# iostanin1/SCTL

Hardware: AMD Instinct MI355X
Metric: pair-interactions/s, Laplace-SL N x N direct sum (higher is better)
Workload: dtype f64; 1 GPU; Laplace3D single layer (Laplace3D-FxU), 2^20 x 2^20, fp64 [BASELINE headline / north_star target]; kernel=Laplace3D-FxU, n_trg=1048576, n_src=1048576, digits=-1

## Files before the change

sctl_amd/csrc/centered.hip:

```cpp
#include "centered_kernel.hpp"
#include "centered_mfma_kernel.hpp"
#include <sctl_amd/device/launch.hpp>
#include "workspace.hpp"

#include <cstdlib>

#include <rocprim/device/device_radix_sort.hpp>

namespace sctl_amd {

#define CENTERED_TRY(expr)            \
  do {                                \
    hipError_t e_ = (expr);           \
    if (e_ != hipSuccess) return e_;  \
  } while (0)


namespace {
bool use_mfma_f32() {
  const char* e = std::getenv("SCTL_AMD_MFMA_F32");
  return !(e && e[0] == '0');
}
}
int centered_pipe(int kernel_id, int real, int mode) {
  const bool has = kernel_id == Laplace3D_FxU::ID || kernel_id == Laplace3D_DxU::ID || kernel_id == Stokes3D_FxU::ID || kernel_id == Stokes3D_FSxU::ID ||
                   kernel_id == Stokes3D_FxUP::ID || kernel_id == Stokes3D_DxU::ID || kernel_id == Stokes3D_FxT::ID || kernel_id == Laplace3D_FxdU::ID || kernel_id == Laplace3D_FDxUdU::ID;
  return (has && real == 1  && mode == 0 && use_mfma_f32()) ? 2 : 1;
}
int centered_targets_per_wave(int kernel_id, int real, int mode, int64_t density) {
  if (centered_pipe(kernel_id, real, mode) != 2) {
    if (kernel_id == Laplace3D_FxdU::ID) return 64 * CenteredFxdU<double>::targets_per_lane<double>();
    if (kernel_id == Stokes3D_FxUP::ID) return 64 * CenteredStokeslet<double, Stokes3D_FxUP>::targets_per_lane<double>();
    return 64 * (real == 0  ? CenteredFxU<double>::targets_per_lane<double>() : CenteredFxU<float>::targets_per_lane<float>());
  }
  if (const char* e = (kernel_id == Laplace3D_FxU::ID || kernel_id == Laplace3D_DxU::ID) ? std::getenv("SCTL_AMD_MFMA_CB") : nullptr) {
    if (e[0] == '8') return 256;
    if (e[0] == '4') return 128;
  }
  if (kernel_id != Laplace3D_FxU::ID && kernel_id != Laplace3D_DxU::ID) return 128;
  return (kernel_id == Laplace3D_FxU::ID && density < ((int64_t)1 << 20)) ? 128 : 256;
}
namespace {
template <class R> struct CenteredStresslet { using Ker = Stokes3D_DxU; };
template <class CP> struct mfma_moments_policy { using type = void; };
template <class KER> struct mfma_moments_policy<CenteredStokeslet<float, KER>> { using type = MfmaStokeslet<KER>; };
template <> struct mfma_moments_policy<CenteredStresslet<float>> { using type = MfmaStresslet; };
template <class R> struct CenteredTraction { using Ker = Stokes3D_FxT; };
template <class R> struct CenteredFusedLaplace { using Ker = Laplace3D_FDxUdU; };
template <> struct mfma_moments_policy<CenteredFusedLaplace<float>> { using type = MfmaFusedLaplace; };
template <> struct mfma_moments_policy<CenteredFxdU<float>> { using type = MfmaGradient; };
template <> struct mfma_moments_policy<CenteredTraction<float>> { using type = MfmaTraction; };
template <class CP, class R, int MODE> void launch_centered(const EvalArgs<R>& a, dim3 grid, int per_wave, hipStream_t st) {
  using MP = typename mfma_moments_policy<CP>::type;
  if constexpr (std::is_same<R, float>::value && !std::is_void<MP>::value) {
    if constexpr (MODE == 0) hipLaunchKernelGGL((centered_mfma_moments_f32_kernel<MP>), grid, dim3(kWaveBlock), 0, st, a);
    return;
  } else {
  if constexpr (std::is_same<R, float>::value && MODE == 0) {
    if (use_mfma_f32()) {
      constexpr bool DL = std::is_same<CP, CenteredDxU<float>>::value;
      if (per_wave == 256) {
        if constexpr (DL) hipLaunchKernelGGL((centered_mfma_f32_kernel<true, 8>), grid, dim3(kWaveBlock), 0, st, a);
        else hipLaunchKernelGGL(centered_mfma_fxu256_f32_kernel, grid, dim3(kWaveBlock), 0, st, a);
      } else {
        hipLaunchKernelGGL((centered_mfma_f32_kernel<DL, 4>), grid, dim3(kWaveBlock), 0, st, a);
      }
      return;
    }
  }
  hipLaunchKernelGGL((centered_kernel<CP, R, MODE, CP::template targets_per_lane<R>()>), grid, dim3(kWaveBlock), 0, st, a);
  }
}
}

void centered_plan(int64_t Nt, int64_t Ns, int cus, int src_bytes, int out_bytes, int* T, int* splits, int64_t* chunk) {
  *T = 2;
  const int64_t wg_x = (Nt + kWaveBlock * 2 - 1) / (kWaveBlock * 2);
  const int64_t want = (int64_t)cus * 16 * 64;
  const int64_t ntile = (Ns + kWaveTile - 1) / kWaveTile;
  int64_t s = (want + wg_x - 1) / wg_x;
  const int64_t s_l2 = (Ns * src_bytes + (2 << 20) - 1) / (2 << 20);
  if (s < s_l2) s = s_l2;
  if (s > ntile / 64) s = ntile / 64;
  if (s > 8) s = (s + 7) & ~(int64_t)7;
  if (s > 256) s = 256;
  {
    const int64_t fit = ((int64_t)2 << 30) / (Nt * out_bytes > 0 ? Nt * out_bytes : 1);
    if (s > fit) s = (fit >= 8) ? (fit & ~(int64_t)7) : fit;
  }
  if (s < 1) s = 1;
  const int64_t tiles_per = (ntile + s - 1) / s;
  *chunk = tiles_per * kWaveTile;
  *splits = (int)((Ns + *chunk - 1) / *chunk);
}

template <class CP, class R>
hipError_t eval_centered_t(int64_t Nt, int64_t Ns, const R* xt, const R* xs, const R* xn, const R* f, R* v_trg, double scale_d, int mode, int cus,
                           hipStream_t st, bool presorted, int64_t density) {
  const R scale = (R)scale_d;
  constexpr int K1 = CP::Ker::K1;
  int T, splits;
  int64_t chunk;
  centered_plan(Nt, Ns, cus, (int)sizeof(R) * (3 + CP::Ker::ND + CP::Ker::K0), (int)sizeof(R) * K1, &T, &splits, &chunk);
  if (presorted) {
    R* partial = nullptr;
    if (splits > 1) {
      void* base = nullptr;
      CENTERED_TRY(workspace_acquire(st, sizeof(R) * (size_t)splits * (size_t)Nt * K1, &base));
      partial = (R*)base;
    }
    EvalArgs<R> a{};
    a.Nt = Nt; a.Ns = Ns; a.xt = xt; a.xs = xs; a.xn = xn; a.f = f; a.v_trg = v_trg; a.partial = partial;
    a.chunk = chunk; a.scale = scale;
    a.ctx.v[0] = kNearFactor2;
    const int64_t per_wave = centered_targets_per_wave(CP::Ker::ID, sizeof(R) == 8 ? 0 : 1, mode, density);
    const dim3 grid((unsigned)((Nt + per_wave - 1) / per_wave), (unsigned)splits);
    if (mode == 0) launch_centered<CP, R, 0>(a, grid, (int)per_wave, st);
    else if (mode == 1) launch_centered<CP, R, 1>(a, grid, (int)per_wave, st);
    else launch_centered<CP, R, (sizeof(R) == 8 ? 2 : 1)>(a, grid, (int)per_wave, st);
    CENTERED_TRY(hipGetLastError());
    if (splits > 1)
      hipLaunchKernelGGL((reduce_splits_kernel<R>), dim3((unsigned)((Nt * K1 + kBlock - 1) / kBlock)), dim3(kBlock), 0, st, v_trg, (const R*)partial, Nt * K1, splits, scale);
    return hipGetLastError();
  }
  const int nblk_box = 256;
  const unsigned nb = (unsigned)((Nt + kBlock - 1) / kBlock);
  size_t tmp_bytes = 0;
  CENTERED_TRY(rocprim::radix_sort_pairs(nullptr, tmp_bytes, (uint64_t*)nullptr, (uint64_t*)nullptr, (uint32_t*)nullptr, (uint32_t*)nullptr, (size_t)Nt, 0,
                                         63, st));
  const size_t n = (size_t)Nt;
  const size_t total = Carver::pad(sizeof(double) * 6 * nblk_box) + 2 * Carver::pad(sizeof(uint64_t) * n) + 2 * Carver::pad(sizeof(uint32_t) * n) +
                       Carver::pad(sizeof(R) * 3 * n) + Carver::pad(sizeof(R) * n * K1) + Carver::pad(tmp_bytes) +
                       (splits > 1 ? Carver::pad(sizeof(R) * (size_t)splits * n * K1) : 0);
  void* base = nullptr;
  CENTERED_TRY(workspace_acquire(st, total, &base));
  Carver cut(base);
  double* part = cut.take<double>(6 * nblk_box);
  uint64_t *keys = cut.take<uint64_t>(n), *keys2 = cut.take<uint64_t>(n);
  uint32_t *idx = cut.take<uint32_t>(n), *idx2 = cut.take<uint32_t>(n);
  R *xts = cut.take<R>(3 * n), *outs = cut.take<R>(n * K1);
  char* tmp = cut.take<char>(tmp_bytes);
  R* partial = (splits > 1) ? cut.take<R>((size_t)splits * n * K1) : nullptr;

  hipLaunchKernelGGL((bbox_partial_kernel<R>), dim3(nblk_box), dim3(kBlock), 0, st, xt, Nt, part);
  hipLaunchKernelGGL((morton_keys_kernel<R>), dim3(nb), dim3(kBlock), 0, st, xt, Nt, (const double*)part, nblk_box, keys, idx);
  CENTERED_TRY(rocprim::radix_sort_pairs(tmp, tmp_bytes, keys, keys2, idx, idx2, (size_t)Nt, 0, 63, st));
  const uint32_t* perm = idx2;
  hipLaunchKernelGGL((gather_points_kernel<R>), dim3(nb), dim3(kBlock), 0, st, xt, perm, Nt, xts);
  CENTERED_TRY(hipMemsetAsync(outs, 0, sizeof(R) * Nt * K1, st));

  EvalArgs<R> a{};
  a.Nt = Nt; a.Ns = Ns; a.xt = xts; a.xs = xs; a.xn = xn; a.f = f; a.v_trg = outs; a.partial = nullptr;
  a.chunk = chunk; a.scale = scale;
  a.ctx.v[0] = kNearFactor2;
  a.partial = partial;
  const int64_t per_wave = centered_targets_per_wave(CP::Ker::ID, sizeof(R) == 8 ? 0 : 1, mode, density);
  const dim3 grid((unsigned)((Nt + per_wave - 1) / per_wave), (unsigned)splits);
  if (mode == 0) launch_centered<CP, R, 0>(a, grid, (int)per_wave, st);
  else if (mode == 1) launch_centered<CP, R, 1>(a, grid, (int)per_wave, st);
  else launch_centered<CP, R, (sizeof(R) == 8 ? 2 : 1)>(a, grid, (int)per_wave, st);
  CENTERED_TRY(hipGetLastError());
  if (splits > 1)
    hipLaunchKernelGGL((reduce_splits_kernel<R>), dim3((unsigned)((Nt * K1 + kBlock - 1) / kBlock)), dim3(kBlock), 0, st, outs, (const R*)a.partial, Nt * K1, splits, scale);
  hipLaunchKernelGGL((scatter_add_kernel<R>), dim3(nb), dim3(kBlock), 0, st, (const R*)outs, perm, Nt, K1, v_trg);
  return hipGetLastError();
}
template <class R> hipError_t morton_order_device_t(const R* d_x, int64_t n, R* d_sorted, uint32_t* d_perm, hipStream_t st) {
  if (n <= 0) return hipSuccess;
  const int nblk_box = 256;
  const unsigned nb = (unsigned)((n + kBlock - 1) / kBlock);
  size_t tmp_bytes = 0;
  CENTERED_TRY(rocprim::radix_sort_pairs(nullptr, tmp_bytes, (uint64_t*)nullptr, (uint64_t*)nullptr, (uint32_t*)nullptr, (uint32_t*)nullptr, (size_t)n, 0, 63, st));
  const size_t total = Carver::pad(sizeof(double) * 6 * nblk_box) + 2 * Carver::pad(sizeof(uint64_t) * (size_t)n) + Carver::pad(sizeof(uint32_t) * (size_t)n) + Carver::pad(tmp_bytes);
  void* base = nullptr;
  CENTERED_TRY(workspace_acquire(st, total, &base));
  Carver cut(base);
  double* part = cut.take<double>(6 * nblk_box);
  uint64_t *keys = cut.take<uint64_t>((size_t)n), *keys2 = cut.take<uint64_t>((size_t)n);
  uint32_t* idx = cut.take<uint32_t>((size_t)n);
  char* tmp = cut.take<char>(tmp_bytes);
  hipLaunchKernelGGL((bbox_partial_kernel<R>), dim3(nblk_box), dim3(kBlock), 0, st, d_x, n, part);
  hipLaunchKernelGGL((morton_keys_kernel<R>), dim3(nb), dim3(kBlock), 0, st, d_x, n, (const double*)part, nblk_box, keys, idx);
  CENTERED_TRY(rocprim::radix_sort_pairs(tmp, tmp_bytes, keys, keys2, idx, d_perm, (size_t)n, 0, 63, st));
  hipLaunchKernelGGL((gather_points_kernel<R>), dim3(nb), dim3(kBlock), 0, st, d_x, (const uint32_t*)d_perm, n, d_sorted);
  return hipGetLastError();
}
hipError_t morton_order_device(int real, const void* d_x, int64_t n, void* d_sorted, uint32_t* d_perm, hipStream_t st) {
  return real == 0  ? morton_order_device_t<double>((const double*)d_x, n, (double*)d_sorted, d_perm, st)
                              : morton_order_device_t<float>((const float*)d_x, n, (float*)d_sorted, d_perm, st);
}

template <class R>
hipError_t eval_centered(int kernel_id, int64_t Nt, int64_t Ns, const R* xt, const R* xs, const R* xn, const R* f, R* v_trg, double scale, int mode, int cus,
                         hipStream_t st, bool presorted, int64_t density) {
  if (kernel_id == Laplace3D_DxU::ID) return eval_centered_t<CenteredDxU<R>, R>(Nt, Ns, xt, xs, xn, f, v_trg, scale, mode, cus, st, presorted, density);
  if constexpr (std::is_same<R, double>::value) {
    if (kernel_id == Laplace3D_FxdU::ID) return eval_centered_t<CenteredFxdU<R>, R>(Nt, Ns, xt, xs, xn, f, v_trg, scale, mode, cus, st, presorted, density);
    if (kernel_id == Stokes3D_FxUP::ID) return eval_centered_t<CenteredStokeslet<R, Stokes3D_FxUP>, R>(Nt, Ns, xt, xs, xn, f, v_trg, scale, mode, cus, st, presorted, density);
  }
  if constexpr (std::is_same<R, float>::value) {
    if (kernel_id == Laplace3D_FxdU::ID) return eval_centered_t<CenteredFxdU<R>, R>(Nt, Ns, xt, xs, xn, f, v_trg, scale, mode, cus, st, presorted, density);
    if (kernel_id == Laplace3D_FDxUdU::ID) return eval_centered_t<CenteredFusedLaplace<R>, R>(Nt, Ns, xt, xs, xn, f, v_trg, scale, mode, cus, st, presorted, density);
    if (kernel_id == Stokes3D_FxU::ID) return eval_centered_t<CenteredStokeslet<R, Stokes3D_FxU>, R>(Nt, Ns, xt, xs, xn, f, v_trg, scale, mode, cus, st, presorted, density);
    if (kernel_id == Stokes3D_FSxU::ID) return eval_centered_t<CenteredStokeslet<R, Stokes3D_FSxU>, R>(Nt, Ns, xt, xs, xn, f, v_trg, scale, mode, cus, st, presorted, density);
    if (kernel_id == Stokes3D_FxUP::ID) return eval_centered_t<CenteredStokeslet<R, Stokes3D_FxUP>, R>(Nt, Ns, xt, xs, xn, f, v_trg, scale, mode, cus, st, presorted, density);
    if (kernel_id == Stokes3D_DxU::ID) return eval_centered_t<CenteredStresslet<R>, R>(Nt, Ns, xt, xs, xn, f, v_trg, scale, mode, cus, st, presorted, density);
    if (kernel_id == Stokes3D_FxT::ID) return eval_centered_t<CenteredTraction<R>, R>(Nt, Ns, xt, xs, xn, f, v_trg, scale, mode, cus, st, presorted, density);
  }
  return eval_centered_t<CenteredFxU<R>, R>(Nt, Ns, xt, xs, xn, f, v_trg, scale, mode, cus, st, presorted, density);
}
template hipError_t eval_centered<double>(int, int64_t, int64_t, const double*, const double*, const double*, const double*, double*, double, int, int, hipStream_t, bool, int64_t);
template hipError_t eval_centered<float>(int, int64_t, int64_t, const float*, const float*, const float*, const float*, float*, double, int, int, hipStream_t, bool, int64_t);

}
```

sctl_amd/csrc/centered_kernel.hpp:

```cpp
#pragma once
#include <sctl_amd/device/eval_kernel.hpp>
#include "curve_key.hpp"

namespace sctl_amd {

constexpr double kNearFactor2 = 4.0;

template <class R> __device__ __forceinline__ R wave_min(R v) {
  for (int o = 32; o > 0; o >>= 1) { const R w = __shfl_xor(v, o); v = (w < v) ? w : v; }
  return v;
}
template <class R> __device__ __forceinline__ R wave_max(R v) {
  for (int o = 32; o > 0; o >>= 1) { const R w = __shfl_xor(v, o); v = (w > v) ? w : v; }
  return v;
}

__device__ __forceinline__ double uniform_(double v) {
  return __hiloint2double(__builtin_amdgcn_readfirstlane(__double2hiint(v)), __builtin_amdgcn_readfirstlane(__double2loint(v)));
}
__device__ __forceinline__ float uniform_(float v) { return __int_as_float(__builtin_amdgcn_readfirstlane(__float_as_int(v))); }
__device__ __forceinline__ double sqrt_(double v) { return __builtin_sqrt(v); }
__device__ __forceinline__ float sqrt_(float v) { return __builtin_sqrtf(v); }

template <class R> struct Rec4;
template <> struct Rec4<double> {
  typedef double V __attribute__((ext_vector_type(2)));
  static constexpr int NW = 2;
  static __device__ __forceinline__ void put(V* p, double a, double b, double c, double d) { p[0] = V{a, b}; p[1] = V{c, d}; }
  static __device__ __forceinline__ void get(const V* p, double (&o)[4]) { const V u = p[0], w = p[1]; o[0] = u[0]; o[1] = u[1]; o[2] = w[0]; o[3] = w[1]; }
};
template <> struct Rec4<float> {
  typedef float V __attribute__((ext_vector_type(4)));
  static constexpr int NW = 1;
  static __device__ __forceinline__ void put(V* p, float a, float b, float c, float d) { p[0] = V{a, b, c, d}; }
  static __device__ __forceinline__ void get(const V* p, float (&o)[4]) { const V u = p[0]; o[0] = u[0]; o[1] = u[1]; o[2] = u[2]; o[3] = u[3]; }
};

constexpr int kWaveBlock = 64;
constexpr int kWaveTile = 64;
#if defined(SCTL_AMD_EXPERIMENTS) && defined(SCTL_AMD_EXP_NEARCAP)
constexpr int kNearCap = SCTL_AMD_EXP_NEARCAP;
static_assert(kNearCap >= 64, "a tile of 64 sources must fit the list of pending near sources");
#else
constexpr int kNearCap = 128;
#endif

typedef float f32x2 __attribute__((ext_vector_type(2)));
template <int MODE, int P = 1> __device__ __forceinline__ f32x2 rsqrt_pair(f32x2 r2) {
  f32x2 y = {__builtin_amdgcn_rsqf(r2[0]), __builtin_amdgcn_rsqf(r2[1])};
  if (MODE >= 1) {
    const f32x2 a = r2 * y;
    y = y * (f32x2{3.0f, 3.0f} - a * y);
    if (MODE == 2) {
      const float k = (float)__builtin_pow(rsqrt_pow_factor(2, P), 1.0 / P) / 2;
      y = y * f32x2{k, k};
    }
  }
  return y;
}
__device__ __forceinline__ f32x2 pk_add_hi(f32x2 t, f32x2 zA) {
  f32x2 r;
  asm("v_pk_add_f32 %0, %1, %2 op_sel:[0,1] op_sel_hi:[1,1]" : "=v"(r) : "v"(t), "v"(zA));
  return r;
}
__device__ __forceinline__ f32x2 pk_fma_lo_hi(f32x2 m, f32x2 g) {
  f32x2 r;
  asm("v_pk_fma_f32 %0, %1, %2, %2 op_sel:[0,0,1] op_sel_hi:[1,0,1]" : "=v"(r) : "v"(m), "v"(g));
  return r;
}

template <class R, int T> struct FarTargets {
  R m2x[T][3], tt[T];
  __device__ __forceinline__ void set(int j, const R (&p)[3], R t2) {
    tt[j] = t2;
#pragma unroll
    for (int k = 0; k < 3; k++) m2x[j][k] = R(-2) * p[k];
  }
};
template <> struct FarTargets<float, 2> {
  f32x2 mp[3], tp;
  __device__ __forceinline__ void set(int j, const float (&p)[3], float t2) {
    tp[j] = t2;
#pragma unroll
    for (int k = 0; k < 3; k++) mp[k][j] = -2.0f * p[k];
  }
};

template <class R> struct CenteredFxU {
  using Ker = Laplace3D_FxU;
  static constexpr bool DUP = std::is_same<R, float>::value;
  static constexpr int XW = DUP ? 2 : 1, NF = 1, NEAR_CAP = 128;
  template <class RR> static constexpr int targets_per_lane() { return sizeof(RR) == 8 ? 4 : 2; }
  struct Extra { R f, f2; };
  template <int MODE> static __device__ __forceinline__ void put_extra(R* base, int q, const R (&)[3], const R*, const R* f) {
    if (DUP) { base[2 * q] = f[0]; base[2 * q + 1] = f[0]; }
    else base[q] = f[0];
  }
  static __device__ __forceinline__ void put_null(R* base, int q) {
    if (DUP) { base[2 * q] = R(0); base[2 * q + 1] = R(0); }
    else base[q] = R(0);
  }
  static __device__ __forceinline__ Extra load_extra(const R* base, int s) { return DUP ? Extra{base[2 * s], base[2 * s + 1]} : Extra{base[s], R(0)}; }
  static __device__ __forceinline__ void store_extra(R* base, int q, const Extra& e) {
    if (DUP) { base[2 * q] = e.f; base[2 * q + 1] = e.f2; }
    else base[q] = e.f;
  }
  static constexpr bool FOLD = !DUP;
  static __device__ __forceinline__ int fold_class(R f, R ss, R& k) {
    if (f == R(0)) return 0;
    k = R(1) / (f * f);
    const R kss = k * ss;
    if (!(kss >= R(0x1p-600) && kss <= R(0x1p600) && ss >= R(0x1p-300) && ss <= R(0x1p300))) return 2;
    return f > R(0) ? 1 : -1;
  }
  static __device__ __forceinline__ void put_folded(typename Rec4<R>::V* rec, R* base, int q, const R (&p)[3], R ss, R k) {
    Rec4<R>::put(rec + q * Rec4<R>::NW, k * p[0], k * p[1], k * p[2], k * ss);
    base[q] = k;
  }
  template <int MODE> static __device__ __forceinline__ void far_pair(R& acc, const R (&m2x)[3], R tt, const R (&b)[4], const Extra& e, const RsqConst<R>& K) {
    const R r2 = fma_(m2x[0], b[0], fma_(m2x[1], b[1], fma_(m2x[2], b[2], tt + b[3])));
    acc = fma_(e.f, rsqrt_scaled<MODE, false>(r2, K), acc);
  }
  template <int MODE, bool NEG> static __device__ __forceinline__ void far_pair_folded(R& acc, const R (&m2x)[3], R tt, const R (&b)[4], const Extra& e,
                                                                                       const RsqConst<R>& K) {
    const R r2 = fma_(m2x[0], b[0], fma_(m2x[1], b[1], fma_(m2x[2], b[2], fma_(tt, e.f, b[3]))));
    const RsqSplit<R> s = rsqrt_scaled_split<MODE, false>(r2, K);
    acc = fma_(NEG ? -s.y : s.y, s.p, acc);
  }
  template <int MODE, int T, bool NEG = false, class KC> static __device__ __forceinline__ void far_pairs(R (&acc)[T][NF], const FarTargets<R, T>& tg, const R (&b)[4],
                                                                                                          const Extra& e, const KC& K) {
    if constexpr (FOLD) {
#pragma unroll
      for (int j = 0; j < T; j++) far_pair_folded<MODE, NEG>(acc[j][0], tg.m2x[j], tg.tt[j], b, e, K.rsq);
    } else if constexpr (std::is_same<R, float>::value && T == 2) {
      f32x2 r2 = pk_add_hi(tg.tp, f32x2{b[2], b[3]});
      r2 = tg.mp[2] * f32x2{b[2], b[2]} + r2;
      r2 = tg.mp[1] * f32x2{b[1], b[1]} + r2;
      r2 = tg.mp[0] * f32x2{b[0], b[0]} + r2;
      const f32x2 a = f32x2{acc[0][0], acc[1][0]} + f32x2{e.f, e.f2} * rsqrt_pair<MODE>(r2);
      acc[0][0] = a[0]; acc[1][0] = a[1];
    } else {
#pragma unroll
      for (int j = 0; j < T; j++) far_pair<MODE>(acc[j][0], tg.m2x[j], tg.tt[j], b, e, K.rsq);
    }
  }
};
template <class R> struct CenteredDxU {
  using Ker = Laplace3D_DxU;
  static constexpr int XW = 4, NF = 1, NEAR_CAP = 128;
  template <class RR> static constexpr int targets_per_lane() { return sizeof(RR) == 8 ? 4 : 2; }
  struct Extra { R g[4]; };
  template <int MODE> static __device__ __forceinline__ void put_extra(R* base, int q, const R (&p)[3], const R* n, const R* f) {
    const R nf[3] = {n[0] * f[0], n[1] * f[0], n[2] * f[0]};
    Rec4<R>::put((typename Rec4<R>::V*)base + q * Rec4<R>::NW, R(-0.5) * nf[0], R(-0.5) * nf[1], R(-0.5) * nf[2], -(p[0] * nf[0] + p[1] * nf[1] + p[2] * nf[2]));
  }
  static __device__ __forceinline__ void put_null(R* base, int q) { Rec4<R>::put((typename Rec4<R>::V*)base + q * Rec4<R>::NW, R(0), R(0), R(0), R(0)); }
  static __device__ __forceinline__ Extra load_extra(const R* base, int s) {
    Extra e;
    Rec4<R>::get((const typename Rec4<R>::V*)base + s * Rec4<R>::NW, e.g);
    return e;
  }
  static __device__ __forceinline__ void store_extra(R* base, int q, const Extra& e) {
    Rec4<R>::put((typename Rec4<R>::V*)base + q * Rec4<R>::NW, e.g[0], e.g[1], e.g[2], e.g[3]);
  }
  template <int MODE> static __device__ __forceinline__ void far_pair(R& acc, const R (&m2x)[3], R tt, const R (&b)[4], const Extra& e, const RsqConst<R>& K) {
    const R r2 = fma_(m2x[0], b[0], fma_(m2x[1], b[1], fma_(m2x[2], b[2], tt + b[3])));
    const R y3 = rsqrt_pow_scaled<MODE, 3, false>(r2, K);
    const R dn = fma_(m2x[0], e.g[0], fma_(m2x[1], e.g[1], fma_(m2x[2], e.g[2], e.g[3])));
    acc = fma_(dn, y3, acc);
  }
  template <int MODE, int T, class KC> static __device__ __forceinline__ void far_pairs(R (&acc)[T][NF], const FarTargets<R, T>& tg, const R (&b)[4], const Extra& e,
                                                                                          const KC& K) {
    if constexpr (std::is_same<R, float>::value && T == 2) {
      const f32x2 mx = tg.mp[0], my = tg.mp[1], mz = tg.mp[2];
      f32x2 r2 = pk_add_hi(tg.tp, f32x2{b[2], b[3]});
      r2 = mz * f32x2{b[2], b[2]} + r2;
      r2 = my * f32x2{b[1], b[1]} + r2;
      r2 = mx * f32x2{b[0], b[0]} + r2;
      const f32x2 y = rsqrt_pair<MODE, 3>(r2);
      f32x2 dn = pk_fma_lo_hi(mz, f32x2{e.g[2], e.g[3]});
      dn = my * f32x2{e.g[1], e.g[1]} + dn;
      dn = mx * f32x2{e.g[0], e.g[0]} + dn;
      const f32x2 a = f32x2{acc[0][0], acc[1][0]} + dn * (y * y * y);
      acc[0][0] = a[0]; acc[1][0] = a[1];
    } else {
#pragma unroll
      for (int j = 0; j < T; j++) far_pair<MODE>(acc[j][0], tg.m2x[j], tg.tt[j], b, e, K.rsq);
    }
  }
};

template <class R, int XW> struct ExtraWords {
  static_assert(XW % 4 == 0, "whole Rec4 groups");
  struct Extra { R g[XW]; };
  static __device__ __forceinline__ Extra load_extra(const R* base, int s) {
    Extra e;
#pragma unroll
// ... 11 lines not shown
  }
  static __device__ __forceinline__ void put_null(R* base, int q) {
    Extra e;
#pragma unroll
    for (int k = 0; k < XW; k++) e.g[k] = R(0);
    store_extra(base, q, e);
  }
};
template <class R> struct CenteredFxdU : ExtraWords<R, 4> {
  using Ker = Laplace3D_FxdU;
  using Extra = typename ExtraWords<R, 4>::Extra;
  static constexpr int XW = 4, NF = 4, NEAR_CAP = 128;
  template <class RR> static constexpr int targets_per_lane() { return 3; }
  template <int MODE> static __device__ __forceinline__ void put_extra(R* base, int q, const R (&p)[3], const R*, const R* f) {
    Extra e{{f[0], f[0] * p[0], f[0] * p[1], f[0] * p[2]}};
    ExtraWords<R, 4>::store_extra(base, q, e);
  }
  template <int MODE, int T, class KC> static __device__ __forceinline__ void far_pairs(R (&acc)[T][NF], const FarTargets<R, T>& tg, const R (&b)[4], const Extra& e,
                                                                                          const KC& K) {
#pragma unroll
    for (int j = 0; j < T; j++) {
      const R r2 = fma_(tg.m2x[j][0], b[0], fma_(tg.m2x[j][1], b[1], fma_(tg.m2x[j][2], b[2], tg.tt[j] + b[3])));
      const R y3 = rsqrt_pow_scaled<MODE, 3, false>(r2, K.rsq);
#pragma unroll
      for (int k = 0; k < 4; k++) acc[j][k] = fma_(y3, e.g[k], acc[j][k]);
    }
  }
  template <int MODE> static __device__ __forceinline__ void finish(R (&out)[3], const R (&far)[NF], const R (&near)[3], const R (&m2x)[3]) {
#pragma unroll
    for (int k = 0; k < 3; k++) out[k] = near[k] + fma_(R(-0.5) * m2x[k], far[0], -far[1 + k]);
  }
};
template <class R, class KER> struct CenteredStokeslet : ExtraWords<R, 8> {
  using Ker = KER;
  using Extra = typename ExtraWords<R, 8>::Extra;
  static constexpr int XW = 8, NF = 4, NEAR_CAP = 64;
  static_assert(KER::K0 == 3 || KER::K0 == 4, "three force components, optionally a source/sink strength");
  static_assert(KER::K1 == 3 || KER::K1 == 4, "velocity, optionally the pressure");
  template <class RR> static constexpr int targets_per_lane() { return 4; }
  template <int MODE> static __device__ __forceinline__ void put_extra(R* base, int q, const R (&p)[3], const R*, const R* f) {
    const R c2 = R(rsqrt_scaled_c2(MODE));
    R g3 = -(p[0] * f[0] + p[1] * f[1] + p[2] * f[2]);
    if constexpr (KER::K0 == 4) g3 += f[3];
    Extra e{{R(-0.5) * f[0], R(-0.5) * f[1], R(-0.5) * f[2], g3, c2 * f[0], c2 * f[1], c2 * f[2], R(0)}};
    ExtraWords<R, 8>::store_extra(base, q, e);
  }
  template <int MODE, int T, class KC> static __device__ __forceinline__ void far_pairs(R (&acc)[T][NF], const FarTargets<R, T>& tg, const R (&b)[4], const Extra& e,
                                                                                          const KC& K) {
#pragma unroll
    for (int j = 0; j < T; j++) {
      const R r2 = fma_(tg.m2x[j][0], b[0], fma_(tg.m2x[j][1], b[1], fma_(tg.m2x[j][2], b[2], tg.tt[j] + b[3])));
      const R y = rsqrt_scaled<MODE, false>(r2, K.rsq);
      const R t = fma_(tg.m2x[j][0], e.g[0], fma_(tg.m2x[j][1], e.g[1], fma_(tg.m2x[j][2], e.g[2], e.g[3]))) * (y * y);
      acc[j][3] = fma_(t, y, acc[j][3]);
#pragma unroll
      for (int k = 0; k < 3; k++) acc[j][k] = fma_(y, fma_(-t, b[k], e.g[4 + k]), acc[j][k]);
    }
  }
  template <int MODE> static __device__ __forceinline__ void finish(R (&out)[KER::K1], const R (&far)[NF], const R (&near)[KER::K1], const R (&m2x)[3]) {
#pragma unroll
    for (int k = 0; k < 3; k++) out[k] = near[k] + fma_(R(-0.5) * m2x[k], far[3], far[k]);
    if constexpr (KER::K1 == 4) out[3] = near[3] + far[3];
  }
};

__device__ __forceinline__ void centered_tile_and_split(unsigned& tile_idx, unsigned& split_idx) {
  tile_idx = blockIdx.x; split_idx = blockIdx.y;
  if ((gridDim.y & 7u) == 0) {
    const unsigned b = blockIdx.y * gridDim.x + blockIdx.x, xcd = b & 7u, j = b >> 3, per = gridDim.y >> 3;
    tile_idx = j % gridDim.x;
    split_idx = xcd * per + j / gridDim.x;
  }
}
template <class CP, class = void> struct FoldsDensity : std::false_type {};
template <class CP> struct FoldsDensity<CP, std::void_t<decltype(CP::FOLD)>> : std::integral_constant<bool, CP::FOLD> {};

template <class CP, class R, int MODE, int T, int UNR = 4>
__global__ void __launch_bounds__(kWaveBlock) centered_kernel(const EvalArgs<R> a) {
  using V = typename Rec4<R>::V;
  constexpr int NW = Rec4<R>::NW;
  using Ker = typename CP::Ker;
  constexpr int ND = Ker::ND, K0 = Ker::K0, K1 = Ker::K1, NF = CP::NF;
  constexpr bool SCALAR = (K1 == 1 && NF == 1);
  constexpr int kNearCap = CP::NEAR_CAP < sctl_amd::kNearCap ? CP::NEAR_CAP : sctl_amd::kNearCap;
  constexpr int NEARW = (Ker::NREC + 3) / 4;
  constexpr int XV = (CP::XW * (int)sizeof(R) + 15) / 16;
  constexpr bool FOLD = FoldsDensity<CP>::value;
  constexpr int FAR_CAP = FOLD ? kWaveTile + 2 * (UNR - 1) : kWaveTile + UNR;
  __shared__ V farB[FAR_CAP * NW];
  __shared__ V farXv[FAR_CAP * (XV > 0 ? XV : 1)];
  __shared__ V nearA[(kNearCap + 2) * NW * NEARW];
  R* const farX = (R*)farXv;

  const int lane = threadIdx.x;
  unsigned tile_idx, split_idx;
  centered_tile_and_split(tile_idx, split_idx);
  const int64_t tbase = (int64_t)tile_idx * (kWaveBlock * T);
  const typename Ker::template Consts<R> K(nullptr);

  R xt[T][3];
  R c[3];
  {
    R lo[3] = {max_finite<R>(), max_finite<R>(), max_finite<R>()}, hi[3] = {-lo[0], -lo[0], -lo[0]};
#pragma unroll
    for (int j = 0; j < T; j++) {
      int64_t t = tbase + j * kWaveBlock + lane;
      if (t >= a.Nt) t = a.Nt - 1;
#pragma unroll
      for (int k = 0; k < 3; k++) {
        xt[j][k] = a.xt[t * 3 + k];
        lo[k] = (xt[j][k] < lo[k]) ? xt[j][k] : lo[k];
        hi[k] = (xt[j][k] > hi[k]) ? xt[j][k] : hi[k];
      }
    }
#pragma unroll
    for (int k = 0; k < 3; k++) c[k] = uniform_(R(0.5) * wave_min(lo[k]) + R(0.5) * wave_max(hi[k]));
  }
  FarTargets<R, T> tg;
  R rt2 = 0;
#pragma unroll
  for (int j = 0; j < T; j++) {
    const R p[3] = {xt[j][0] - c[0], xt[j][1] - c[1], xt[j][2] - c[2]};
    const R t2 = len2(p);
    rt2 = (t2 > rt2) ? t2 : rt2;
    tg.set(j, p, t2);
  }
  rt2 = uniform_(wave_max(rt2));
  const R near_r2 = R(a.ctx.v[0]) * rt2;

  R acc[T][K1];
  R facc[T][SCALAR ? 1 : NF];
#pragma unroll
  for (int j = 0; j < T; j++) {
#pragma unroll
    for (int k = 0; k < K1; k++) acc[j][k] = 0;
#pragma unroll
    for (int k = 0; k < (SCALAR ? 1 : NF); k++) facc[j][k] = 0;
  }

  const int64_t s_begin = (int64_t)split_idx * a.chunk;
  const int64_t s_end = (s_begin + a.chunk < a.Ns) ? s_begin + a.chunk : a.Ns;
  const int64_t len = (s_end > s_begin) ? s_end - s_begin : 0;
  const int ntile = (int)((len + kWaveTile - 1) / kWaveTile);

  R x[3] = {0, 0, 0}, nrm[3] = {0, 0, 0}, f[K0];
#pragma unroll
  for (int k = 0; k < K0; k++) f[k] = 0;
  auto load_source = [&](int it) {
    const int64_t s = s_begin + (int64_t)it * kWaveTile + lane;
    if (s < s_end) {
#pragma unroll
      for (int k = 0; k < 3; k++) x[k] = a.xs[s * 3 + k];
#pragma unroll
      for (int k = 0; k < ND; k++) nrm[k] = a.xn[s * ND + k];
#pragma unroll
      for (int k = 0; k < K0; k++) f[k] = a.f[s * K0 + k];
    }
  };
  if (ntile > 0) load_source(0);

  const R far_off = R(1.0e3) * (R(1) + sqrt_(rt2));
  auto put_near = [&](int q, const R (&xq)[3], const R (&nq)[3], const R (&fq)[K0]) {
    R rec[4 * NEARW] = {};
    pack_record<Ker, R, MODE>(rec, xq, nq, fq);
#pragma unroll
    for (int g = 0; g < NEARW; g++) Rec4<R>::put(nearA + (q * NEARW + g) * NW, rec[4 * g], rec[4 * g + 1], rec[4 * g + 2], rec[4 * g + 3]);
  };
  int nn = 0;
  auto flush_near = [&]() {
    if (nn & 1) {
      if (lane == 0) {
        const R xq[3] = {c[0] + far_off, c[1], c[2]}, nq[3] = {0, 0, 0}, fq[K0] = {};
        put_near(nn, xq, nq, fq);
      }
      __syncthreads();
    }
    R xo[T][3];
#pragma unroll
    for (int j = 0; j < T; j++) {
      int64_t t = tbase + j * kWaveBlock + lane;
      if (t >= a.Nt) t = a.Nt - 1;
#pragma unroll
      for (int k = 0; k < 3; k++) xo[j][k] = a.xt[t * 3 + k];
    }
    for (int s = 0; s < nn; s += 2) {
#pragma unroll
      for (int u = 0; u < 2; u++) {
        R q[4 * NEARW];
#pragma unroll
        for (int g = 0; g < NEARW; g++) {
          R w[4];
          Rec4<R>::get(nearA + ((s + u) * NEARW + g) * NW, w);
          q[4 * g] = w[0]; q[4 * g + 1] = w[1]; q[4 * g + 2] = w[2]; q[4 * g + 3] = w[3];
        }
#pragma unroll
        for (int j = 0; j < T; j++) {
          const R d[3] = {xo[j][0] - q[0], xo[j][1] - q[1], xo[j][2] - q[2]};
          Ker::template pair<R, MODE, true>(acc[j], d, q, a.ctx, K);
#if !(defined(SCTL_AMD_EXPERIMENTS) && defined(SCTL_AMD_EXP_NO_NEAR_FENCE))
          __builtin_amdgcn_sched_barrier(0);
#endif
        }
      }
    }
    nn = 0;
  };

  auto stage_tile = [&](int it, int carry) -> int {
    const int ns = (it == ntile - 1) ? (int)(len - (int64_t)it * kWaveTile) : kWaveTile;
    const bool valid = lane < ns;
    const R p[3] = {x[0] - c[0], x[1] - c[1], x[2] - c[2]};
    const R ss = len2(p);
    const bool is_far = valid && (ss > near_r2);
    const bool is_near = valid && !is_far;
    const unsigned long long bf = __ballot(is_far), bn = __ballot(is_near);
    const unsigned long long below = (lane == 0) ? 0ull : (~0ull >> (64 - lane));
    const int nfar = __popcll(bf), nnear = __popcll(bn);
    __syncthreads();
    if (nn + nnear > kNearCap) {
      flush_near();
      __syncthreads();
    }
    if (is_far) {
      const int q = carry + __popcll(bf & below);
      Rec4<R>::put(farB + q * NW, p[0], p[1], p[2], ss);
      CP::template put_extra<MODE>(farX, q, p, nrm, f);
    } else if (is_near) {
      put_near(nn + __popcll(bn & below), x, nrm, f);
    }
    nn += nnear;
    return nfar;
  };
  auto run_far = [&](int m) {
    R tacc[T][NF];
#pragma unroll
    for (int j = 0; j < T; j++)
#pragma unroll
      for (int k = 0; k < NF; k++) tacc[j][k] = 0;
    for (int s = 0; s < m; s += UNR) {
#pragma unroll
      for (int u = 0; u < UNR; u++) {
        R b[4];
        Rec4<R>::get(farB + (s + u) * NW, b);
        const typename CP::Extra e = CP::load_extra(farX, s + u);
        CP::template far_pairs<MODE, T>(tacc, tg, b, e, K);
      }
    }
#pragma unroll
    for (int j = 0; j < T; j++) {
      if constexpr (SCALAR) acc[j][0] += tacc[j][0];
      else {
#pragma unroll
        for (int k = 0; k < NF; k++) facc[j][k] += tacc[j][k];
      }
    }
  };
  auto put_null_far = [&](int q) { Rec4<R>::put(farB + q * NW, far_off, R(0), R(0), far_off * far_off); CP::put_null(farX, q); };

  if constexpr (FOLD) {
    static_assert(SCALAR && NF == 1, "the fold is the single layer's");
    auto stage_tile_folded = [&](int it, int cpos, int cneg, int& npos, int& nneg) {
      const int ns = (it == ntile - 1) ? (int)(len - (int64_t)it * kWaveTile) : kWaveTile;
      const bool valid = lane < ns;
      const R p[3] = {x[0] - c[0], x[1] - c[1], x[2] - c[2]};
      const R ss = len2(p);
      const bool far = valid && (ss > near_r2);
      R k = 0;
      const int cls = far ? CP::fold_class(f[0], ss, k) : 2;
      const bool is_pos = far && cls == 1, is_neg = far && cls == -1, is_near = valid && cls == 2;
      const unsigned long long bp = __ballot(is_pos), bq = __ballot(is_neg), bn = __ballot(is_near);
      const unsigned long long below = (lane == 0) ? 0ull : (~0ull >> (64 - lane));
      const int nnear = __popcll(bn);
      __syncthreads();
      if (nn + nnear > kNearCap) {
        flush_near();
        __syncthreads();
      }
      if (is_pos) CP::put_folded(farB, farX, cpos + __popcll(bp & below), p, ss, k);
      else if (is_neg) CP::put_folded(farB, farX, FAR_CAP - 1 - (cneg + __popcll(bq & below)), p, ss, k);
      else if (is_near) put_near(nn + __popcll(bn & below), x, nrm, f);
      nn += nnear;
      npos = __popcll(bp);
      nneg = __popcll(bq);
    };
    auto far_folded = [&](R (&tacc)[T][NF], int i, auto neg) {
      constexpr bool NEG = decltype(neg)::value;
      const int q = NEG ? FAR_CAP - 1 - i : i;
      R b[4];
      Rec4<R>::get(farB + q * NW, b);
      const typename CP::Extra e = CP::load_extra(farX, q);
      CP::template far_pairs<MODE, T, NEG>(tacc, tg, b, e, K);
    };
    auto run_far_folded = [&](int mp, int mn) {
      R tacc[T][NF];
#pragma unroll
      for (int j = 0; j < T; j++) tacc[j][0] = 0;
      const std::integral_constant<bool, false> pos;
      const std::integral_constant<bool, true> neg;
      const int mb = mp < mn ? mp : mn;
      int s = 0;
      for (; s < mb; s += UNR) {
#pragma unroll
        for (int u = 0; u < UNR; u++) far_folded(tacc, s + u, pos);
#pragma unroll
        for (int u = 0; u < UNR; u++) far_folded(tacc, s + u, neg);
      }
      for (; s < mp; s += UNR) {
#pragma unroll
        for (int u = 0; u < UNR; u++) far_folded(tacc, s + u, pos);
      }
      for (; s < mn; s += UNR) {
#pragma unroll
        for (int u = 0; u < UNR; u++) far_folded(tacc, s + u, neg);
      }
#pragma unroll
      for (int j = 0; j < T; j++) acc[j][0] += tacc[j][0];
    };
    int cpos = 0, cneg = 0;
    for (int it = 0; it < ntile; it++) {
      int npos, nneg;
      stage_tile_folded(it, cpos, cneg, npos, nneg);
      const int np = cpos + npos, nq = cneg + nneg, mp = np & ~(UNR - 1), mq = nq & ~(UNR - 1);
      if (it + 1 < ntile) load_source(it + 1);
      __syncthreads();
      run_far_folded(mp, mq);
      cpos = np - mp;
      cneg = nq - mq;
      const bool mv_pos = mp > 0 && lane < cpos, mv_neg = mq > 0 && lane >= 32 && lane < 32 + cneg;
      if (mv_pos || mv_neg) {
        const int from = mv_pos ? mp + lane : FAR_CAP - 1 - (mq + lane - 32), to = mv_pos ? lane : FAR_CAP - 1 - (lane - 32);
        R b[4];
        Rec4<R>::get(farB + from * NW, b);
        const typename CP::Extra e = CP::load_extra(farX, from);
        Rec4<R>::put(farB + to * NW, b[0], b[1], b[2], b[3]);
        CP::store_extra(farX, to, e);
      }
    }
    __syncthreads();
    if (cpos + cneg > 0) {
      R tacc[T][NF];
#pragma unroll
      for (int j = 0; j < T; j++) tacc[j][0] = 0;
      for (int i = 0; i < cpos; i++) far_folded(tacc, i, std::integral_constant<bool, false>());
      for (int i = 0; i < cneg; i++) far_folded(tacc, i, std::integral_constant<bool, true>());
#pragma unroll
      for (int j = 0; j < T; j++) acc[j][0] += tacc[j][0];
    }
  } else if constexpr (sizeof(R) == 8) {
    int carry = 0;
    for (int it = 0; it < ntile; it++) {
      const int n = carry + stage_tile(it, carry), m = n & ~(UNR - 1);
      if (it + 1 < ntile) load_source(it + 1);
      __syncthreads();
      run_far(m);
      carry = n - m;
      if (m > 0 && lane < carry) {
        R b[4];
        Rec4<R>::get(farB + (m + lane) * NW, b);
        const typename CP::Extra e = CP::load_extra(farX, m + lane);
        Rec4<R>::put(farB + lane * NW, b[0], b[1], b[2], b[3]);
        CP::store_extra(farX, lane, e);
      }
    }
    __syncthreads();
    if (carry > 0) {
      if (lane < UNR - carry) put_null_far(carry + lane);
      __syncthreads();
      run_far(UNR);
    }
  } else {
    for (int it = 0; it < ntile; it++) {
      const int nfar = stage_tile(it, 0), padded = (nfar + UNR - 1) & ~(UNR - 1);
      if (lane < UNR - 1 && nfar + lane < padded) put_null_far(nfar + lane);
      if (it + 1 < ntile) load_source(it + 1);
      __syncthreads();
      run_far(padded);
    }
  }
  __syncthreads();
  flush_near();

#pragma unroll
  for (int j = 0; j < T; j++) {
    const int64_t t = tbase + j * kWaveBlock + lane;
    if constexpr (SCALAR) {
      if (t < a.Nt) {
        if (gridDim.y == 1) a.v_trg[t] += acc[j][0] * a.scale;
        else a.partial[(int64_t)split_idx * a.Nt + t] = acc[j][0];
      }
    } else {
      R out[K1];
      CP::template finish<MODE>(out, facc[j], acc[j], tg.m2x[j]);
      finish_acc<Ker, R, MODE>(out);
      if (t < a.Nt) {
#pragma unroll
        for (int k = 0; k < K1; k++) {
          if (gridDim.y == 1) a.v_trg[t * K1 + k] += out[k] * a.scale;
          else a.partial[((int64_t)split_idx * a.Nt + t) * K1 + k] = out[k];
        }
      }
    }
  }
}

template <class R> __global__ void __launch_bounds__(kBlock) bbox_partial_kernel(const R* x, int64_t n, double* part) {
  __shared__ double red[4 * 6];
  double lo[3] = {1.7976931348623157e308, 1.7976931348623157e308, 1.7976931348623157e308}, hi[3] = {-lo[0], -lo[0], -lo[0]};
  for (int64_t i = (int64_t)blockIdx.x * kBlock + threadIdx.x; i < n; i += (int64_t)gridDim.x * kBlock) {
#pragma unroll
    for (int k = 0; k < 3; k++) {
      const double v = (double)x[i * 3 + k];
      lo[k] = (v < lo[k]) ? v : lo[k];
      hi[k] = (v > hi[k]) ? v : hi[k];
    }
  }
#pragma unroll
  for (int k = 0; k < 3; k++) { lo[k] = wave_min(lo[k]); hi[k] = wave_max(hi[k]); }
  const int lane = threadIdx.x & 63, wave = threadIdx.x >> 6;
  if (lane == 0) {
#pragma unroll
    for (int k = 0; k < 3; k++) { red[wave * 6 + k] = lo[k]; red[wave * 6 + 3 + k] = hi[k]; }
  }
  __syncthreads();
  if (threadIdx.x < 6) {
    const int k = threadIdx.x;
    double v = red[k];
    for (int w = 1; w < 4; w++) v = (k < 3) ? ((red[w * 6 + k] < v) ? red[w * 6 + k] : v) : ((red[w * 6 + k] > v) ? red[w * 6 + k] : v);
    part[blockIdx.x * 6 + k] = v;
  }
}

template <class R> __global__ void __launch_bounds__(kBlock) morton_keys_kernel(const R* x, int64_t n, const double* part, int nblk, uint64_t* keys, uint32_t* idx) {
  __shared__ double box[6];
  if (threadIdx.x < 6) {
    const int k = threadIdx.x;
    double v = part[k];
    for (int b = 1; b < nblk; b++) v = (k < 3) ? ((part[b * 6 + k] < v) ? part[b * 6 + k] : v) : ((part[b * 6 + k] > v) ? part[b * 6 + k] : v);
    box[k] = v;
  }
  __syncthreads();
  const int64_t i = (int64_t)blockIdx.x * kBlock + threadIdx.x;
  if (i >= n) return;
  const double p[3] = {(double)x[i * 3], (double)x[i * 3 + 1], (double)x[i * 3 + 2]};
  keys[i] = curve_key(p, box);
  idx[i] = (uint32_t)i;
}

template <class R> __global__ void __launch_bounds__(kBlock) gather_points_kernel(const R* x, const uint32_t* perm, int64_t n, R* out) {
  const int64_t i = (int64_t)blockIdx.x * kBlock + threadIdx.x;
  if (i >= n) return;
  const int64_t s = perm[i];
#pragma unroll
  for (int k = 0; k < 3; k++) out[i * 3 + k] = x[s * 3 + k];
}

template <class R> __global__ void __launch_bounds__(kBlock) scatter_add_kernel(const R* sorted, const uint32_t* perm, int64_t n, int k1, R* v_trg) {
  const int64_t i = (int64_t)blockIdx.x * kBlock + threadIdx.x;
  if (i >= n) return;
  const int64_t t = perm[i];
  for (int k = 0; k < k1; k++) v_trg[t * k1 + k] += sorted[i * k1 + k];
}

}
```

Measured before the change: 3013 billion pair-interactions/s.

## Precompute sign-partitioned folded source records in a per-split prepass kernel

Adds a prepass kernel that classifies each source by density sign, precomputes the fold factor k=1/f^2, and writes compacted positive and negative source records (x,y,z,k) into per-split tiles, with exceptional sources listed separately. The main fp64 single-layer kernel then streams these pre-sorted records instead of loading raw sources and classifying them per target wave. This removes redundant per-tile classification, division and ballot work, and lets it skip the sync/flush in the common case where a whole tile is far. The cost is an extra kernel launch, extra workspace, and a larger shared-memory far buffer and near cap, which may reduce occupancy.

```diff
diff --git a/sctl_amd/csrc/centered.hip b/sctl_amd/csrc/centered.hip
--- a/sctl_amd/csrc/centered.hip
+++ b/sctl_amd/csrc/centered.hip
@@ -94,6 +94,11 @@
   *splits = (int)((Ns + *chunk - 1) / *chunk);
 }
 
+template <class R> const R* fold_prepass(const R* xs, const R* f, int64_t Ns, int splits, int64_t chunk, char* blk, hipStream_t st) {
+  if constexpr (std::is_same<R, double>::value) hipLaunchKernelGGL(fold_prepass_kernel, dim3((unsigned)splits), dim3(kFoldPrepBlock), 0, st, xs, f, Ns, chunk, blk);
+  return (const R*)blk;
+}
+
 template <class CP, class R>
 hipError_t eval_centered_t(int64_t Nt, int64_t Ns, const R* xt, const R* xs, const R* xn, const R* f, R* v_trg, double scale_d, int mode, int cus,
                            hipStream_t st, bool presorted, int64_t density) {
@@ -102,17 +107,23 @@
   int T, splits;
   int64_t chunk;
   centered_plan(Nt, Ns, cus, (int)sizeof(R) * (3 + CP::Ker::ND + CP::Ker::K0), (int)sizeof(R) * K1, &T, &splits, &chunk);
+  constexpr bool FOLD = FoldsDensity<CP>::value && std::is_same<R, double>::value;
+  const size_t prep_bytes = FOLD ? (size_t)FoldPrepLayout(splits, chunk).bytes : 0;
   if (presorted) {
     R* partial = nullptr;
-    if (splits > 1) {
-      void* base = nullptr;
-      CENTERED_TRY(workspace_acquire(st, sizeof(R) * (size_t)splits * (size_t)Nt * K1, &base));
-      partial = (R*)base;
-    }
+    const size_t partial_bytes = (splits > 1) ? Carver::pad(sizeof(R) * (size_t)splits * (size_t)Nt * K1) : 0;
     EvalArgs<R> a{};
-    a.Nt = Nt; a.Ns = Ns; a.xt = xt; a.xs = xs; a.xn = xn; a.f = f; a.v_trg = v_trg; a.partial = partial;
+    a.Nt = Nt; a.Ns = Ns; a.xt = xt; a.xs = xs; a.xn = xn; a.f = f; a.v_trg = v_trg;
     a.chunk = chunk; a.scale = scale;
     a.ctx.v[0] = kNearFactor2;
+    if (partial_bytes + prep_bytes > 0) {
+      void* base = nullptr;
+      CENTERED_TRY(workspace_acquire(st, partial_bytes + prep_bytes, &base));
+      Carver cut(base);
+      if (splits > 1) partial = cut.take<R>((size_t)splits * (size_t)Nt * K1);
+      if constexpr (FOLD) a.xn = fold_prepass(xs, f, Ns, splits, chunk, cut.take<char>(prep_bytes), st);
+    }
+    a.partial = partial;
     const int64_t per_wave = centered_targets_per_wave(CP::Ker::ID, sizeof(R) == 8 ? 0 : 1, mode, density);
     const dim3 grid((unsigned)((Nt + per_wave - 1) / per_wave), (unsigned)splits);
     if (mode == 0) launch_centered<CP, R, 0>(a, grid, (int)per_wave, st);
@@ -131,7 +142,7 @@
   const size_t n = (size_t)Nt;
   const size_t total = Carver::pad(sizeof(double) * 6 * nblk_box) + 2 * Carver::pad(sizeof(uint64_t) * n) + 2 * Carver::pad(sizeof(uint32_t) * n) +
                        Carver::pad(sizeof(R) * 3 * n) + Carver::pad(sizeof(R) * n * K1) + Carver::pad(tmp_bytes) +
-                       (splits > 1 ? Carver::pad(sizeof(R) * (size_t)splits * n * K1) : 0);
+                       (splits > 1 ? Carver::pad(sizeof(R) * (size_t)splits * n * K1) : 0) + prep_bytes;
   void* base = nullptr;
   CENTERED_TRY(workspace_acquire(st, total, &base));
   Carver cut(base);
@@ -154,6 +165,7 @@
   a.chunk = chunk; a.scale = scale;
   a.ctx.v[0] = kNearFactor2;
   a.partial = partial;
+  if constexpr (FOLD) a.xn = fold_prepass(xs, f, Ns, splits, chunk, cut.take<char>(prep_bytes), st);
   const int64_t per_wave = centered_targets_per_wave(CP::Ker::ID, sizeof(R) == 8 ? 0 : 1, mode, density);
   const dim3 grid((unsigned)((Nt + per_wave - 1) / per_wave), (unsigned)splits);
   if (mode == 0) launch_centered<CP, R, 0>(a, grid, (int)per_wave, st);
diff --git a/sctl_amd/csrc/centered_kernel.hpp b/sctl_amd/csrc/centered_kernel.hpp
--- a/sctl_amd/csrc/centered_kernel.hpp
+++ b/sctl_amd/csrc/centered_kernel.hpp
@@ -1,6 +1,7 @@
 #pragma once
 #include <sctl_amd/device/eval_kernel.hpp>
 #include "curve_key.hpp"
+#include "fold_prepass.hpp"
 
 namespace sctl_amd {
 
@@ -106,13 +107,6 @@
     else base[q] = e.f;
   }
   static constexpr bool FOLD = !DUP;
-  static __device__ __forceinline__ int fold_class(R f, R ss, R& k) {
-    if (f == R(0)) return 0;
-    k = R(1) / (f * f);
-    const R kss = k * ss;
-    if (!(kss >= R(0x1p-600) && kss <= R(0x1p600) && ss >= R(0x1p-300) && ss <= R(0x1p300))) return 2;
-    return f > R(0) ? 1 : -1;
-  }
   static __device__ __forceinline__ void put_folded(typename Rec4<R>::V* rec, R* base, int q, const R (&p)[3], R ss, R k) {
     Rec4<R>::put(rec + q * Rec4<R>::NW, k * p[0], k * p[1], k * p[2], k * ss);
     base[q] = k;
@@ -290,13 +284,14 @@
   using Ker = typename CP::Ker;
   constexpr int ND = Ker::ND, K0 = Ker::K0, K1 = Ker::K1, NF = CP::NF;
   constexpr bool SCALAR = (K1 == 1 && NF == 1);
-  constexpr int kNearCap = CP::NEAR_CAP < sctl_amd::kNearCap ? CP::NEAR_CAP : sctl_amd::kNearCap;
+  constexpr int kNearCap = FoldsDensity<CP>::value ? 144 : (CP::NEAR_CAP < sctl_amd::kNearCap ? CP::NEAR_CAP : sctl_amd::kNearCap);
   constexpr int NEARW = (Ker::NREC + 3) / 4;
   constexpr int XV = (CP::XW * (int)sizeof(R) + 15) / 16;
   constexpr bool FOLD = FoldsDensity<CP>::value;
-  constexpr int FAR_CAP = FOLD ? kWaveTile + 2 * (UNR - 1) : kWaveTile + UNR;
+  constexpr int FAR_CAP = FOLD ? 2 * (kWaveTile + UNR - 1) : kWaveTile + UNR;
   __shared__ V farB[FAR_CAP * NW];
-  __shared__ V farXv[FAR_CAP * (XV > 0 ? XV : 1)];
+  constexpr int FARX_WORDS = FOLD ? (FAR_CAP * CP::XW * (int)sizeof(R) + 15) / 16 : FAR_CAP * (XV > 0 ? XV : 1);
+  __shared__ V farXv[FARX_WORDS];
   __shared__ V nearA[(kNearCap + 2) * NW * NEARW];
   R* const farX = (R*)farXv;
 
@@ -365,7 +360,9 @@
       for (int k = 0; k < K0; k++) f[k] = a.f[s * K0 + k];
     }
   };
-  if (ntile > 0) load_source(0);
+  if constexpr (!FOLD) {
+    if (ntile > 0) load_source(0);
+  }
 
   const R far_off = R(1.0e3) * (R(1) + sqrt_(rt2));
   auto put_near = [&](int q, const R (&xq)[3], const R (&nq)[3], const R (&fq)[K0]) {
@@ -466,30 +463,43 @@
   auto put_null_far = [&](int q) { Rec4<R>::put(farB + q * NW, far_off, R(0), R(0), far_off * far_off); CP::put_null(farX, q); };
 
   if constexpr (FOLD) {
-    static_assert(SCALAR && NF == 1, "the fold is the single layer's");
-    auto stage_tile_folded = [&](int it, int cpos, int cneg, int& npos, int& nneg) {
-      const int ns = (it == ntile - 1) ? (int)(len - (int64_t)it * kWaveTile) : kWaveTile;
-      const bool valid = lane < ns;
+    static_assert(SCALAR && NF == 1 && std::is_same<R, double>::value, "the fold is the fp64 single layer's");
+    static_assert(ND == 0 && K0 == 1, "a.xn is free to carry the pre-pass block");
+    const FoldPrepLayout L((int64_t)gridDim.y, a.chunk);
+    const char* const blk = (const char*)a.xn;
+    const int32_t* const hdr = (const int32_t*)blk + 4 * (int64_t)split_idx;
+    const int npt = hdr[0], nnt = hdr[1], nexc = hdr[2];
+    const int cap = (int)L.cap;
+    const V* const rec = (const V*)(blk + L.rec) + (int64_t)split_idx * cap * NW;
+    const uint32_t* const ridx = (const uint32_t*)(blk + L.idx) + (int64_t)split_idx * cap;
+    const uint32_t* const exc = (const uint32_t*)(blk + L.exc) + (int64_t)split_idx * a.chunk;
+    R kf = 0;
+    auto load_rec = [&](int r0) {
+      const R* const w = (const R*)(rec + (int64_t)r0 * NW) + lane * 4;
+      x[0] = w[0]; x[1] = w[1]; x[2] = w[2]; kf = w[3];
+    };
+    auto stage_rec = [&](int r0, int carry, auto neg) -> int {
+      constexpr bool NEG = decltype(neg)::value;
       const R p[3] = {x[0] - c[0], x[1] - c[1], x[2] - c[2]};
-      const R ss = len2(p);
-      const bool far = valid && (ss > near_r2);
-      R k = 0;
-      const int cls = far ? CP::fold_class(f[0], ss, k) : 2;
-      const bool is_pos = far && cls == 1, is_neg = far && cls == -1, is_near = valid && cls == 2;
-      const unsigned long long bp = __ballot(is_pos), bq = __ballot(is_neg), bn = __ballot(is_near);
-      const unsigned long long below = (lane == 0) ? 0ull : (~0ull >> (64 - lane));
+      const R ss = len2(p), kss = kf * ss;
+      const bool valid = kf != R(0);
+      const bool far = valid && ss > near_r2 && kss >= R(0x1p-600) && kss <= R(0x1p600) && ss >= R(0x1p-300) && ss <= R(0x1p300);
+      const unsigned long long bv = __ballot(valid), bf = __ballot(far);
+      if (bf == bv) {
+        if (valid) CP::put_folded(farB, farX, NEG ? FAR_CAP - 1 - (carry + lane) : carry + lane, p, ss, kf);
+        return __popcll(bv);
+      }
+      const unsigned long long bn = bv & ~bf, below = (lane == 0) ? 0ull : (~0ull >> (64 - lane));
       const int nnear = __popcll(bn);
-      __syncthreads();
-      if (nn + nnear > kNearCap) {
-        flush_near();
-        __syncthreads();
-      }
-      if (is_pos) CP::put_folded(farB, farX, cpos + __popcll(bp & below), p, ss, k);
-      else if (is_neg) CP::put_folded(farB, farX, FAR_CAP - 1 - (cneg + __popcll(bq & below)), p, ss, k);
-      else if (is_near) put_near(nn + __popcll(bn & below), x, nrm, f);
+      if (far) {
+        const int q = carry + __popcll(bf & below);
+        CP::put_folded(farB, farX, NEG ? FAR_CAP - 1 - q : q, p, ss, kf);
+      } else if (valid) {
+        const R fq[K0] = {a.f[s_begin + ridx[r0 + lane]]};
+        put_near(nn + __popcll(bn & below), x, nrm, fq);
+      }
       nn += nnear;
-      npos = __popcll(bp);
-      nneg = __popcll(bq);
+      return __popcll(bf);
     };
     auto far_folded = [&](R (&tacc)[T][NF], int i, auto neg) {
       constexpr bool NEG = decltype(neg)::value;
@@ -524,12 +534,27 @@
 #pragma unroll
       for (int j = 0; j < T; j++) acc[j][0] += tacc[j][0];
     };
+    const std::integral_constant<bool, false> pos;
+    const std::integral_constant<bool, true> neg;
+    const int nstep = npt > nnt ? npt : nnt;
     int cpos = 0, cneg = 0;
-    for (int it = 0; it < ntile; it++) {
-      int npos, nneg;
-      stage_tile_folded(it, cpos, cneg, npos, nneg);
+    if (nstep > 0) load_rec((int)fold_prep_tile_base(npt == 0, 0, cap));
+    for (int it = 0; it < nstep; it++) {
+      const bool hp = it < npt, hn = it < nnt;
+      int npos = 0, nneg = 0;
+      __syncthreads();
+      if (hp) {
+        npos = stage_rec(it * kWaveTile, cpos, pos);
+        if (hn) load_rec((int)fold_prep_tile_base(true, it, cap));
+      }
+      if (hn) nneg = stage_rec((int)fold_prep_tile_base(true, it, cap), cneg, neg);
+      if (nn > kNearCap - 2 * kWaveTile) {
+        __syncthreads();
+        flush_near();
+      }
+      if (it + 1 < npt) load_rec((it + 1) * kWaveTile);
+      else if (it + 1 < nnt) load_rec((int)fold_prep_tile_base(true, it + 1, cap));
       const int np = cpos + npos, nq = cneg + nneg, mp = np & ~(UNR - 1), mq = nq & ~(UNR - 1);
-      if (it + 1 < ntile) load_source(it + 1);
       __syncthreads();
       run_far_folded(mp, mq);
       cpos = np - mp;
@@ -549,10 +574,24 @@
       R tacc[T][NF];
 #pragma unroll
       for (int j = 0; j < T; j++) tacc[j][0] = 0;
-      for (int i = 0; i < cpos; i++) far_folded(tacc, i, std::integral_constant<bool, false>());
-      for (int i = 0; i < cneg; i++) far_folded(tacc, i, std::integral_constant<bool, true>());
+      for (int i = 0; i < cpos; i++) far_folded(tacc, i, pos);
+      for (int i = 0; i < cneg; i++) far_folded(tacc, i, neg);
 #pragma unroll
       for (int j = 0; j < T; j++) acc[j][0] += tacc[j][0];
+    }
+    for (int e0 = 0; e0 < nexc; e0 += kWaveTile) {
+      const int ne = (nexc - e0 < kWaveTile) ? nexc - e0 : kWaveTile;
+      if (nn + ne > kNearCap) {
+        __syncthreads();
+        flush_near();
+        __syncthreads();
+      }
+      if (lane < ne) {
+        const int64_t s = s_begin + exc[e0 + lane];
+        const R xq[3] = {a.xs[s * 3], a.xs[s * 3 + 1], a.xs[s * 3 + 2]}, fq[K0] = {a.f[s]};
+        put_near(nn + lane, xq, nrm, fq);
+      }
+      nn += ne;
     }
   } else if constexpr (sizeof(R) == 8) {
     int carry = 0;
@@ -611,6 +650,62 @@
   }
 }
 
+constexpr int kFoldPrepBlock = 1024;
+__global__ void __launch_bounds__(kFoldPrepBlock) fold_prepass_kernel(const double* xs, const double* f, int64_t Ns, int64_t chunk, char* blk) {
+  constexpr int NWAVE = kFoldPrepBlock / 64;
+  __shared__ int cnt[2][3][NWAVE];
+  const int tid = threadIdx.x, lane = tid & 63, wave = tid >> 6;
+  const int64_t split = blockIdx.x;
+  const FoldPrepLayout L((int64_t)gridDim.x, chunk);
+  double* const rec = (double*)(blk + L.rec) + split * L.cap * 4;
+  uint32_t* const idx = (uint32_t*)(blk + L.idx) + split * L.cap;
+  uint32_t* const exc = (uint32_t*)(blk + L.exc) + split * chunk;
+  const int64_t s_begin = split * chunk;
+  const int64_t s_end = (s_begin + chunk < Ns) ? s_begin + chunk : Ns;
+  const int len = (int)((s_end > s_begin) ? s_end - s_begin : 0);
+  const unsigned long long below = (lane == 0) ? 0ull : (~0ull >> (64 - lane));
+  int npos = 0, nneg = 0, nexc = 0;
+  for (int off = 0, step = 0; off < len; off += kFoldPrepBlock, step++) {
+    const int o = off + tid;
+    double k;
+    const int cls = fold_prep_class(o < len ? f[s_begin + o] : 0.0, k);
+    const unsigned long long bp = __ballot(cls == 1), bq = __ballot(cls == -1), be = __ballot(cls == 2);
+    int (*const cn)[NWAVE] = cnt[step & 1];
+    if (lane == 0) { cn[0][wave] = __popcll(bp); cn[1][wave] = __popcll(bq); cn[2][wave] = __popcll(be); }
+    __syncthreads();
+    int before_p = 0, before_q = 0, before_e = 0, tot_p = 0, tot_q = 0, tot_e = 0;
+#pragma unroll
+    for (int w = 0; w < NWAVE; w++) {
+      const int vp = cn[0][w], vq = cn[1][w], ve = cn[2][w];
+      tot_p += vp; tot_q += vq; tot_e += ve;
+      if (w < wave) { before_p += vp; before_q += vq; before_e += ve; }
+    }
+    if (cls == 1 || cls == -1) {
+      const bool neg = cls == -1;
+      const int rank = neg ? nneg + before_q + __popcll(bq & below) : npos + before_p + __popcll(bp & below);
+      const int64_t slot = fold_prep_slot(neg, rank, L.cap), s = s_begin + o;
+      rec[slot * 4] = xs[s * 3]; rec[slot * 4 + 1] = xs[s * 3 + 1]; rec[slot * 4 + 2] = xs[s * 3 + 2]; rec[slot * 4 + 3] = k;
+      idx[slot] = (uint32_t)o;
+    } else if (cls == 2) {
+      exc[nexc + before_e + __popcll(be & below)] = (uint32_t)o;
+    }
+    npos += tot_p; nneg += tot_q; nexc += tot_e;
+  }
+#pragma unroll
+  for (int sgn = 0; sgn < 2; sgn++) {
+    const int n = sgn ? nneg : npos, fill = (int)fold_prep_tiles(n) * kFoldTile - n;
+    if (tid < fill) {
+      const int64_t slot = fold_prep_slot(sgn == 1, n + tid, L.cap);
+      rec[slot * 4] = 0; rec[slot * 4 + 1] = 0; rec[slot * 4 + 2] = 0; rec[slot * 4 + 3] = 0;
+      idx[slot] = 0;
+    }
+  }
+  if (tid == 0) {
+    int32_t* const hdr = (int32_t*)blk + 4 * split;
+    hdr[0] = (int32_t)fold_prep_tiles(npos); hdr[1] = (int32_t)fold_prep_tiles(nneg); hdr[2] = nexc; hdr[3] = 0;
+  }
+}
+
 template <class R> __global__ void __launch_bounds__(kBlock) bbox_partial_kernel(const R* x, int64_t n, double* part) {
   __shared__ double red[4 * 6];
   double lo[3] = {1.7976931348623157e308, 1.7976931348623157e308, 1.7976931348623157e308}, hi[3] = {-lo[0], -lo[0], -lo[0]};
diff --git a/sctl_amd/csrc/fold_prepass.hpp b/sctl_amd/csrc/fold_prepass.hpp
--- /dev/null
+++ b/sctl_amd/csrc/fold_prepass.hpp
@@ -0,0 +1,41 @@
+#pragma once
+#include <cstddef>
+#include <cstdint>
+
+#if defined(__HIPCC__) || defined(__CUDACC__)
+#define SCTL_AMD_FOLD_HD __host__ __device__
+#else
+#define SCTL_AMD_FOLD_HD
+#endif
+
+namespace sctl_amd {
+
+constexpr int kFoldTile = 64;
+
+SCTL_AMD_FOLD_HD inline int fold_prep_class(double f, double& k) {
+  k = 0;
+  if (f == 0.0) return 0;
+  const double kk = 1.0 / (f * f);
+  if (!(kk >= 0x1p-900 && kk <= 0x1p900)) return 2;
+  k = kk;
+  return f > 0.0 ? 1 : -1;
+}
+
+SCTL_AMD_FOLD_HD inline int64_t fold_prep_cap(int64_t chunk) { return chunk + 2 * kFoldTile; }
+SCTL_AMD_FOLD_HD inline int64_t fold_prep_tiles(int64_t n) { return (n + kFoldTile - 1) / kFoldTile; }
+SCTL_AMD_FOLD_HD inline int64_t fold_prep_tile_base(bool neg, int64_t tile, int64_t cap) { return neg ? cap - (tile + 1) * kFoldTile : tile * kFoldTile; }
+SCTL_AMD_FOLD_HD inline int64_t fold_prep_slot(bool neg, int64_t rank, int64_t cap) { return fold_prep_tile_base(neg, rank / kFoldTile, cap) + rank % kFoldTile; }
+
+struct FoldPrepLayout {
+  int64_t cap, rec, idx, exc, bytes;
+  static SCTL_AMD_FOLD_HD int64_t pad(int64_t b) { return (b + 255) & ~(int64_t)255; }
+  SCTL_AMD_FOLD_HD FoldPrepLayout(int64_t splits, int64_t chunk) {
+    cap = fold_prep_cap(chunk);
+    rec = pad(splits * 4 * (int64_t)sizeof(int32_t));
+    idx = rec + pad(splits * cap * 4 * (int64_t)sizeof(double));
+    exc = idx + pad(splits * cap * (int64_t)sizeof(uint32_t));
+    bytes = exc + pad(splits * chunk * (int64_t)sizeof(uint32_t));
+  }
+};
+
+}
```

New measurement: 3045 billion pair-interactions/s (median of 6 runs). +1.0%, better.
